# ylab-hi/ChimeraLM

Measured on AMD Instinct MI355X. Metric: reads/sec (whole node), 8192-bp reads batch=256, higher is better.
Workload: dtype fp16c

## Files before the change

chimeralm_amd/csrc/clm_api.hip:

```cpp
#include <cstdio>
#include <cstdlib>
#include <cmath>
#include <cstring>
#include <map>
#include <algorithm>
#include <string>
#include <vector>

#include "chimeralm_hip.h"
#include "clm_common.h"

using namespace clm;

namespace clm {
bool debug_flag(const char* name) {
    const char* e = std::getenv("CLM_DEBUG");
    if (!e) return false;
    const size_t n = std::strlen(name);
    for (const char* p = e; *p;) {
        const char* q = std::strchr(p, ',');
        const size_t len = q ? (size_t)(q - p) : std::strlen(p);
        if (len == n && std::strncmp(p, name, n) == 0) return true;
        p += len + (q ? 1 : 0);
    }
// ... 348 lines not shown
    *krev_out = nullptr;
    const int S = conv_segments_for(L);
    const int logn = S > 1 ? 14 : conv_logn_for(L);
    if (logn < 0 || L > h->cfg.max_seq_len)
        return fail(h, CLM_E_UNSUPPORTED, "sequence length " + std::to_string(L) + " tokens exceeds max_seq_len " +
                                              std::to_string(h->cfg.max_seq_len));
    const int key = S > 1 ? KEY_LONG : logn;
    FilterSet* fs = nullptr;
    for (auto& f : h->filters)
        if (f.key == key) fs = &f;
    const int N = 1 << logn;
    if (!fs) {
        HIPCHK(h, hipStreamSynchronize(st));
        FilterSet f;
        f.key = key;
        f.logn = logn;
        f.Lf = S > 1 ? h->cfg.max_seq_len : std::min(N / 2 + 1, h->cfg.max_seq_len);
        f.KS = S > 1 ? conv_segments_for(h->cfg.max_seq_len) : 1;
        DevBuf scratch;
        HIPCHK(h, scratch.alloc((size_t)D * N * sizeof(double2)));
        HIPCHK(h, f.tw.alloc((size_t)(N / 2) * sizeof(float2)));
        launch_twiddles(f.tw.get<float2>(), logn, st);
        for (int i = 0; i < NLAYER; ++i) {
            HIPCHK(h, f.ktime[i].alloc((size_t)f.Lf * D * 4));
            HIPCHK(h, f.kf[i].alloc((size_t)D * f.KS * N * sizeof(float2)));
            float* const kt = f.ktime[i].get<float>();
            float2* const kf = f.kf[i].get<float2>();
            const BlockF32& b = h->blk[i];
            launch_filter(b.pos_z, b.pos_t, b.f_w0, b.f_b0, b.f_freq, b.f_w2, b.f_b2, b.f_w4, b.f_b4, b.f_w6, b.deltas, kt, f.Lf, st);
            if (S == 1) {
                launch_filter_spectrum(kt, b.filt_bias, kf, scratch.get<double2>(), f.Lf, logn, 0, f.Lf, -1, st);
                if (logn == 14) {
                    HIPCHK(h, f.kfp[i].alloc((size_t)D * N * sizeof(float2)));
                    launch_spectrum_lanepack(kf, f.kfp[i].get<float2>(), 1, 0, st);
                }
            } else {
                DevBuf tmp;
                HIPCHK(h, tmp.alloc((size_t)D * N * sizeof(float2)));
                for (int j = 0; j < f.KS; ++j) {
                    launch_filter_spectrum(kt, b.filt_bias, tmp.get<float2>(), scratch.get<double2>(), f.Lf, logn, j * SEG_LEN,
                                           SEG_LEN, (j - 1) * SEG_LEN, st);
                    launch_spectrum_lanepack(tmp.get<float2>(), kf, f.KS, j, st);
                }
                HIPCHK(h, hipStreamSynchronize(st));
            }
        }
        HIPCHK(h, hipGetLastError());
        HIPCHK(h, hipStreamSynchronize(st));
        h->filters.push_back(std::move(f));
        fs = &h->filters.back();
    }
    if (conv_lone_tail(L)) {
        for (auto& r : fs->krev)
            if (r.L == L) *krev_out = &r;
        if (!*krev_out) {
            ReversedFilter r;
            r.L = L;
            r.stride = round_up(L, 8);
            for (int i = 0; i < NLAYER; ++i) {
                HIPCHK(h, r.p[i].alloc((size_t)D * r.stride * 4));
                launch_filter_reversed(fs->ktime[i].get<float>(), h->blk[i].filt_bias, r.p[i].get<float>(), L, r.stride, st);
            }
            fs->krev.push_back(std::move(r));
            *krev_out = &fs->krev.back();
        }
    }
    *out = fs;
// ... 442 lines not shown
extern "C" {

int clm_abi_version(void) { return CLM_ABI_VERSION; }

int clm_default_config(clm_config* c) {
    if (!c) return CLM_E_INVALID;
    std::memset(c, 0, sizeof(*c));
    c->struct_size = (int32_t)sizeof(clm_config);
    c->d_model = D; c->n_layer = NLAYER; c->d_inner = DI; c->vocab_rows = VOCAB; c->filter_order = FORDER;
    c->emb_dim = EMB; c->max_seq_len = 32770; c->head_hidden = HH; c->n_classes = NCLS;
    c->ln_eps = 1e-5f;
    c->precision = CLM_PREC_F32;
    c->chunk_reads = 256;
    return CLM_OK;
}

int clm_create(const clm_config* cfg, int device, clm_handle** out) {
    if (!cfg || !out) return fail<clm_handle>(nullptr, CLM_E_INVALID, "clm_create: null argument");
    if (cfg->struct_size != (int32_t)sizeof(clm_config)) return fail<clm_handle>(nullptr, CLM_E_INVALID, "clm_config size mismatch");
    if (cfg->d_model != D || cfg->n_layer != NLAYER || cfg->d_inner != DI || cfg->vocab_rows != VOCAB ||
        cfg->filter_order != FORDER || cfg->emb_dim != EMB || cfg->head_hidden != HH || cfg->n_classes != NCLS)
        return fail<clm_handle>(nullptr, CLM_E_UNSUPPORTED,
                                "only the HyenaDNA-small-32k + 512-wide attention-pooling head of chimeralm/models/lm.py is built");
    if (cfg->precision < CLM_PREC_F32 || cfg->precision > CLM_PREC_F16X3 || cfg->chunk_reads < 1 ||
        cfg->max_seq_len < 2)
        return fail<clm_handle>(nullptr, CLM_E_INVALID, "clm_create: bad precision / chunk_reads / max_seq_len");
    if (int rc = use_gfx950<clm_handle>(device, "clm_create")) return rc;
    clm_handle* h = new clm_handle();
    h->unfused_fp32 = debug_flag("unfused_fp32");
    h->no_idconv = debug_flag("no_idconv");
    h->no_lone_peel = debug_flag("no_lone_peel");
    if (debug_flag("conv_oneshot")) h->conv_flags |= CONV_ONESHOT;
    if (debug_flag("conv_no_xcd")) h->conv_flags |= CONV_NO_XCD;
    h->raw_z = debug_flag("raw_z");
    h->no_pad_skip = debug_flag("no_pad_skip");
    h->no_seg_skip = debug_flag("no_seg_skip");
    h->cfg = *cfg;
    if (cfg->precision == CLM_PREC_F16X3) {
        h->x3 = true;
        h->cfg.precision = CLM_PREC_F32;
        if (h->unfused_fp32) { delete h; return fail<clm_handle>(nullptr, CLM_E_UNSUPPORTED, "CLM_PREC_F16X3 exists in the fused tail kernels only (CLM_DEBUG=unfused_fp32 is set)"); }
    }
    h->device = device;
    if (hipHostMalloc((void**)&h->bad_ids, sizeof(int), hipHostMallocMapped) == hipSuccess) *h->bad_ids = 0;
    else h->bad_ids = nullptr;
    *out = h;
    return CLM_OK;
}

int clm_load_weight(clm_handle* h, const char* key, const void* data, int dtype, const int64_t* shape, int ndim) {
    if (!h || !key || !data || !shape || ndim < 1 || ndim > 4) return fail(h, CLM_E_INVALID, "clm_load_weight: bad argument");
    std::string ck;
    if (!canonical_key(key, ck)) return fail(h, CLM_E_INVALID, std::string("unknown weight key: ") + key);
    if (ck.find("implicit_filter.3.freq") != std::string::npos || ck.find("implicit_filter.5.freq") != std::string::npos)
        return CLM_OK;
    const KeySpec* spec = nullptr;
    static thread_local std::vector<KeySpec> specs;
    specs = expected_keys(h);
    for (auto& s : specs)
        if (s.key == ck) spec = &s;
    if (!spec) return fail(h, CLM_E_INVALID, std::string("unknown weight key: ") + key);
    std::vector<int64_t> shp(shape, shape + ndim);
    if (shp != spec->shape) {
        std::string got, want;
        for (auto v : shp) got += std::to_string(v) + ",";
        for (auto v : spec->shape) want += std::to_string(v) + ",";
// ... 434 lines not shown
```

chimeralm_amd/csrc/clm_common.h:

```cpp
#pragma once
#include <hip/hip_runtime.h>
#include <stdint.h>

#include <array>
#include <atomic>
#include <cstdio>
#include <map>
#include <string>
#include <type_traits>
#include <utility>
#include <vector>

#include "chimeralm_hip.h"

namespace clm {

constexpr int D = 256;
constexpr int D3 = 768;
constexpr int DI = 1024;
constexpr int XCDS = 8;
constexpr int NLAYER = 4;
constexpr int VOCAB = 16;
constexpr int FORDER = 64;
constexpr int EMB = 5;
// ... 387 lines not shown
    const float *n_g, *n_b, *n_w, *n_bias;
    const float4* n_fir;
    const float2* edge_read;
    void* n_z;
    const float *att_w1, *att_b1, *att_w2, *att_b2;
    float *scores, *partial;
    float* ws;
    int B, L, Lp, ntiles;
    float eps;
    const unsigned char* ylo;
    int zlo;
};
size_t lone_token_ws_floats(int B);
void launch_lone_token(int prec, const LoneTokenArgs& a, hipStream_t st);
void launch_tail16(int prec, const TailArgs& m, int next, hipStream_t st);
void tail16_dump_stamps();
void conv_dump_stamps();
size_t packed_weight_bytes(int prec, int n, int k);
void launch_pack_weight(int prec, const float* w, void* out, int n, int k, hipStream_t st);

constexpr int SEG_LEN = 8192;
int conv_logn_for(int L);
int conv_segments_for(int L);
bool conv_lone_tail(int L);
void launch_filter_reversed(const float* k , const float* dskip, float* krev, int L, int stride, hipStream_t st);
void launch_filter(const float* z , const float* t , const float* w0, const float* b0,
                   const float* freq, const float* w2, const float* b2, const float* w4, const float* b4,
                   const float* w6, const float* deltas, float* k_out , int L, hipStream_t st);
void launch_filter_spectrum(const float* k , const float* dskip , float2* kf,
                            double2* scratch, int L, int logn, int seg_off, int seg_len, int prev_off, hipStream_t st);
void launch_twiddles(float2* tw, int logn, hipStream_t st);
constexpr int CONV_ONESHOT = 1;
constexpr int CONV_NO_XCD = 2;
constexpr int CONV_GATED = 4;
void launch_hyena_conv(int prec, const void* z, void* y, const float2* kf, const float2* tw, const float* ktime,
                       const float* short_w, const float* short_b, int B, int L, int Lp, int logn,
                       const unsigned char* ids8, const float* ztab, hipStream_t st, int flags = 0,
                       const float2* kf_packed = nullptr ,
                       unsigned char* ylo = nullptr );
void launch_spectrum_lanepack(const float2* src, float2* dst, int KS, int j, hipStream_t st);
void launch_ztab(const float* emb, const float* g, const float* bta, const float* w, const float* bias, float* ztab,
                 float eps, hipStream_t st);

constexpr int SEG_DOT_THREADS = 512;
struct SegPrefix {
    const int* p0 = nullptr;
    const float2* tab = nullptr;
    int tab_segs = 0;
    const int* perm = nullptr;
    const float* dots_in = nullptr;
    float* dots_out = nullptr;
    int dots_segs = 0;
};
void launch_hyena_conv_seg(int prec, const void* z, void* y, const float2* kf, int KS ,
                           const float2* tw, const float* short_w,
                           const float* short_b, float2* gscratch, int B, int L, int Lp, int S,
                           const float* krev , int krev_stride,
                           const unsigned char* ids8 , const float* ztab,
                           hipStream_t st, int flags = 0, unsigned char* ylo = nullptr ,
                           const SegPrefix& pfx = SegPrefix{});
void launch_spectra_pair_form(float2* table, int S_T, hipStream_t st);

void launch_softmax_stats(const float* scores, float* stats , int B, int L, hipStream_t st);
constexpr int POOL_SPLIT = 16;
void launch_pool(const float* h, const float* g, const float* b, const float* scores, const float* stats,
                 float* partial , int B, int L, float eps, hipStream_t st);
struct HeadW {
    const float *w0t, *b0, *w3t, *b3, *w60t, *b60, *w63t, *b63, *wot, *bo;
};
void launch_head_mlp(const float* partial, const HeadW& hw, float* pooled_out, float* logits, int B, hipStream_t st);
constexpr int POOL_PSTRIDE = 264;
void launch_score_pool16(int prec, const float* h, const float* g, const float* bta, const void* w1, const float* b1,
                         const float* w2, const float* b2, float* scores, float* partial ,
// ... 34 lines not shown
```

chimeralm_amd/csrc/fft_core.h:

```cpp
#pragma once

#if defined(__HIPCC__)
#include <hip/hip_runtime.h>
#define CLM_HD __host__ __device__ __forceinline__
#define CLM_HDC __host__ __device__ constexpr
namespace clmfft {
using V2 = float __attribute__((ext_vector_type(2)));
CLM_HD V2 make_v2(float a, float b) { return V2{a, b}; }
CLM_HD V2 splat2(float a) { return V2{a, a}; }
}
#else
#include <cmath>
#define CLM_HD inline
#define CLM_HDC constexpr
struct float2 {
    float x, y;
};
static inline float2 make_float2(float x, float y) { return float2{x, y}; }
namespace clmfft {
struct V2 {
    float x, y;
};
inline V2 operator+(V2 a, V2 b) { return V2{a.x + b.x, a.y + b.y}; }
inline V2 operator-(V2 a, V2 b) { return V2{a.x - b.x, a.y - b.y}; }
// ... 155 lines not shown
        C t[16];
#pragma unroll
        for (int p = 0; p < 16; ++p) t[p] = v[p];
#pragma unroll
        for (int k1 = 0; k1 < 4; ++k1)
#pragma unroll
            for (int k2 = 0; k2 < 4; ++k2) v[4 * k1 + k2] = t[k1 + 4 * k2];
    }
};

template <bool INV>
struct Dft16HalfOut {
    template <class C>
    static CLM_HD void run(C* v) {
#pragma unroll
        for (int n1 = 0; n1 < 4; ++n1) dft4<INV>(v[n1], v[n1 + 4], v[n1 + 8], v[n1 + 12]);
#pragma unroll
        for (int n1 = 1; n1 < 4; ++n1)
#pragma unroll
            for (int k2 = 1; k2 < 4; ++k2) v[n1 + 4 * k2] = mul_w16<INV>(v[n1 + 4 * k2], n1 * k2);
        C x[9];
#pragma unroll
        for (int k2 = 0; k2 < 4; ++k2) {
            const C a0 = v[4 * k2], a1 = v[4 * k2 + 1], a2 = v[4 * k2 + 2], a3 = v[4 * k2 + 3];
            const C t0 = C::add(a0, a2), t1 = C::sub(a0, a2), t2 = C::add(a1, a3), t3 = C::template mul_mi<INV>(C::sub(a1, a3));
            x[k2] = C::add(t0, t2);
            x[4 + k2] = C::add(t1, t3);
            if (k2 == 0) x[8] = C::sub(t0, t2);
        }
#pragma unroll
        for (int q = 0; q < 9; ++q) v[q] = x[q];
    }
};

template <int R, class C>
CLM_HD void apply_twiddle_powers(C* v, C w1) {
    if (R >= 2) v[1] = C::mul(v[1], w1);
    if (R >= 4) {
        C w2 = C::mul(w1, w1), w3 = C::mul(w2, w1);
        v[2] = C::mul(v[2], w2);
        v[3] = C::mul(v[3], w3);
        if (R >= 8) {
            C w4 = C::mul(w2, w2), w5 = C::mul(w4, w1), w6 = C::mul(w4, w2), w7 = C::mul(w4, w3);
            v[4] = C::mul(v[4], w4);
            v[5] = C::mul(v[5], w5);
            v[6] = C::mul(v[6], w6);
            v[7] = C::mul(v[7], w7);
            if (R >= 16) {
                C w8 = C::mul(w4, w4);
                v[8] = C::mul(v[8], w8);
                v[9] = C::mul(v[9], C::mul(w8, w1));
                v[10] = C::mul(v[10], C::mul(w8, w2));
                v[11] = C::mul(v[11], C::mul(w8, w3));
                v[12] = C::mul(v[12], C::mul(w8, w4));
                v[13] = C::mul(v[13], C::mul(w8, w5));
                v[14] = C::mul(v[14], C::mul(w8, w6));
                v[15] = C::mul(v[15], C::mul(w8, w7));
            }
        }
    }
}

template <int LOGN>
struct Plan {
    static constexpr int N = 1 << LOGN;
    static constexpr int NPASS = (LOGN + 3) / 4;
// ... 31 lines not shown
```

chimeralm_amd/csrc/fft_passes.h:

```cpp
#pragma once
#include "fft_core.h"

namespace clmfft {

template <int LOGN, int R>
struct PassGeom {
    static constexpr int N = 1 << LOGN;
    static constexpr int NB = N / R;
    static constexpr int NT = Plan<LOGN>::NT;
    static constexpr int IT = (NB + NT - 1) / NT;
    static constexpr int NP = (IT + 1) / 2;
    static_assert(NP * R <= 16, "a thread holds at most 16 complex pairs");
    static CLM_HD int jba(int tid, int p) { return tid + (2 * p) * NT; }
    static CLM_HD int jbb(int tid, int p) { return tid + (2 * p + 1) * NT; }
    static constexpr bool FULL = (NB % NT == 0);
    static CLM_HD bool has_a(int tid, int p) { return FULL || jba(tid, p) < NB; }
    static CLM_HD bool has_b(int tid, int p) { return 2 * p + 1 < IT && (FULL || jbb(tid, p) < NB); }
    static_assert(NT % 32 == 0, "lane distance is a whole number of padding periods");
    static CLM_HDC int pb_of(int pa) { return pa + pad_offset(NT); }
};

template <int LOGN, int R>
CLM_HD void pass_load(const float* re, const float* im, Cx2* v, int tid) {
    using G = PassGeom<LOGN, R>;
// ... 103 lines not shown
        const bool ha = G::has_a(tid, p), hb = G::has_b(tid, p);
#pragma unroll
        for (int q = 0; q < R; ++q)
            kv[p * R + q] = pack2(ha ? kf[stockham_in<LOGN, R>(G::jba(tid, p), q)] : zero,
                                  hb ? kf[stockham_in<LOGN, R>(G::jbb(tid, p), q)] : zero);
    }
}

template <int LOGN, int R>
CLM_HD void spectrum_multiply_and_first_inverse_v(Cx2* v, int tid, const Cx2* kv, float tail_re = 0.f, float tail_im = 0.f) {
    using G = PassGeom<LOGN, R>;
    static_assert(((1 << LOGN) / R) % 2 == 0 && G::NT % 2 == 0, "bin parity == thread parity");
    const float sg = (tid & 1) ? -1.f : 1.f;
    const Cx2 tl{splat2(sg * tail_re), splat2(sg * tail_im)};
#pragma unroll
    for (int p = 0; p < G::NP; ++p) {
#pragma unroll
        for (int q = 0; q < R; ++q) v[p * R + q] = Cx2::mul(Cx2::add(v[p * R + q], tl), kv[p * R + q]);
        Dft<R, true>::run(v + p * R);
    }
}

template <int LOGN>
struct TwLayout {
    using P = Plan<LOGN>;
    static constexpr int NP16 = PassGeom<LOGN, 16>::NP;
    static constexpr int NPL = PassGeom<LOGN, P::LAST>::NP;
    static constexpr int fwd(int p) { return (p - 1) * NP16; }
    static constexpr int fwd_last() { return (P::NPASS - 2) * NP16; }
    static constexpr int inv(int p) { return (P::NPASS - 2) * NP16 + NPL + (p - 1) * NP16; }
    static constexpr int TOTAL = (2 * P::NPASS - 3) * NP16 + NPL;
};

}
```

chimeralm_amd/csrc/hyena_conv.hip:

```cpp
#include <cstdio>
#include <cstdlib>
#include <type_traits>
#include <vector>

#include "clm_common.h"
#include "fft_passes.h"

namespace clm {
using namespace clmfft;

__global__ __launch_bounds__(64) void filter_kernel(const float* __restrict__ z, const float* __restrict__ tn,
                                                    const float* __restrict__ w0, const float* __restrict__ b0,
                                                    const float* __restrict__ freq, const float* __restrict__ w2,
                                                    const float* __restrict__ b2, const float* __restrict__ w4,
                                                    const float* __restrict__ b4, const float* __restrict__ w6,
                                                    const float* __restrict__ deltas, float* __restrict__ k_out,
                                                    int L) {
    __shared__ double hbuf[2][FORDER];
    const int t = blockIdx.x, j = threadIdx.x;
    const double f = (double)freq[j];
    double acc = (double)b0[j];
#pragma unroll
    for (int e = 0; e < EMB; ++e) acc += (double)w0[j * EMB + e] * (double)z[(size_t)t * EMB + e];
    hbuf[0][j] = sin(f * acc);
// ... 615 lines not shown
            for (int e = 0; e < 8; ++e) {
                const bool ok = t0 + e < L;
                oA[e] = ok ? oA[e] * x0A[ch][e] : 0.f;
                oB[e] = ok ? oB[e] * x0B[ch][e] : 0.f;
            }
            ystore8<T, LO>(yA + t0, ylA + t0, oA);
            if (hasB) ystore8<T, LO>(yB + t0, ylB + t0, oB);
        }
    }
    if (tail && tid == TAIL_TID) {
        ystore1<T, LO>(yA + HALF, ylA + HALF, bre[pad_index(HALF)] * x0At);
        if (hasB) ystore1<T, LO>(yB + HALF, ylB + HALF, bim[pad_index(HALF)] * x0Bt);
    }
    CLM_STAMP_AT(11);
    if (STAMP && threadIdx.x == 0)
        stamps[((size_t)blockIdx.y * gridDim.x + blockIdx.x) * CONV_NSTAMP + 6] = __builtin_amdgcn_s_memrealtime();
#undef CLM_STAMP_AT
}


template <typename T, bool IDS, bool GATED = false, bool LO = false>
struct ConvGateRaw {
    Raw<T> r[GATED ? 1 : 2][2][GATED ? 1 : 2];
    T ztail[2][2];
    uint2 idd[2][2];
    unsigned short idp[2][2];
    unsigned char idt[2];
    uint4 g[2][2];
    T gtail[2];
    uint2 gl[2][2];
    unsigned char gltail[2];
};

template <typename T, bool IDS, bool GATED = false, bool LO = false>
__global__ __launch_bounds__(Plan<14>::NT) void hyena_conv_pers_kernel(
    const T* __restrict__ z, T* __restrict__ y, const float2* __restrict__ kf , const float2* __restrict__ tw,
    const float* __restrict__ ktime, const float* __restrict__ short_w, const float* __restrict__ short_b, int B, int L,
    int Lp, const unsigned char* __restrict__ ids8, const float* __restrict__ ztab, int use_xcd, unsigned char* __restrict__ ylo) {
    static_assert(!LO || std::is_same<T, f16_t>::value, "lo bytes exist in the compensated fp16 mode only");
    constexpr int LOGN = 14;
    using P = Plan<LOGN>;
    using TL = TwLayout<LOGN>;
    constexpr int N = P::N, NT = P::NT, LAST = P::LAST, HALF = N / 2, CH = 2;
    static_assert(HALF / 8 / NT == CH, "two 8-token chunks per thread");
    constexpr int TAIL_TID = HALF / 8 - 1 - (CH - 1) * NT;
    extern __shared__ __attribute__((aligned(16))) unsigned char smem[];
    float* bre = reinterpret_cast<float*>(smem);
    float* bim = bre + padded_size(N);
    float* gtail = bim + padded_size(N);
    float* zt = gtail + 4;

    const int tid = threadIdx.x;
    const int pairs = (B + 1) / 2, n_units = pairs * D;
    const bool tail = (L == HALF + 1);
    const bool xcd_order = use_xcd && (gridDim.x % XCDS) == 0;
    const int xcd = blockIdx.x % XCDS, wg_in_xcd = blockIdx.x / XCDS, wgs_per_xcd = gridDim.x / XCDS;
    const int first = xcd_order ? wg_in_xcd : (int)blockIdx.x, stride = xcd_order ? wgs_per_xcd : (int)gridDim.x;
    const int n_mine = xcd_order ? n_units / XCDS : n_units;
    auto unit_of = [&](int q, int& c, int& pair) {
        c = xcd_order ? XCDS * (q / pairs) + xcd : q / pairs;
        pair = q % pairs;
    };

    Cx2 wall[TL::TOTAL];
    {
        int ns = 16;
#pragma unroll
        for (int p = 1; p <= P::NPASS - 2; ++p) {
            pass_twiddles<LOGN, 16, false>(wall + TL::fwd(p), tid, ns, tw);
            ns *= 16;
        }
        pass_twiddles<LOGN, LAST, false>(wall + TL::fwd_last(), tid, ns, tw);
        ns = LAST;
#pragma unroll
        for (int p = 1; p <= P::NPASS - 1; ++p) {
            pass_twiddles<LOGN, 16, true>(wall + TL::inv(p), tid, ns, tw);
            ns *= 16;
        }
    }
    static_assert(!(GATED && IDS), "block 0 looks its rows up by token id: nothing to hand over");
    auto request_gate = [&](int q, ConvGateRaw<T, IDS, GATED, LO>& g, int ltid) {
        int c, pair;
        unit_of(q, c, pair);
        const int bA = 2 * pair, bB = (2 * pair + 1 < B) ? 2 * pair + 1 : bA;
        if constexpr (GATED) {
#pragma unroll
            for (int rd = 0; rd < 2; ++rd) {
                const T* row = z + ((size_t)(rd == 0 ? bA : bB) * D3 + D + c) * Lp;
                const unsigned char* rowl = zlo_row(z + (size_t)(rd == 0 ? bA : bB) * D3 * Lp, 1, c, Lp);
#pragma unroll
                for (int ch = 0; ch < CH; ++ch) {
                    const int t0 = 8 * (ltid + ch * NT);
                    g.g[ch][rd] = *reinterpret_cast<const uint4*>(row + (t0 < L ? t0 : 0));
                    if constexpr (LO) g.gl[ch][rd] = *reinterpret_cast<const uint2*>(rowl + (t0 < L ? t0 : 0));
                }
                g.gtail[rd] = row[(tail && ltid == TAIL_TID) ? HALF : 0];
                if constexpr (LO) g.gltail[rd] = rowl[(tail && ltid == TAIL_TID) ? HALF : 0];
            }
// ... 5 lines not shown
                for (int ch = 0; ch < CH; ++ch) {
                    const int t0 = 8 * (ltid + ch * NT);
                    const bool valid = t0 < L;
                    g.idd[ch][rd] = *reinterpret_cast<const uint2*>(ir + (valid ? t0 : 0));
                    g.idp[ch][rd] = *reinterpret_cast<const unsigned short*>(ir + ((valid && t0 > 0) ? t0 - 2 : 0));
                }
                g.idt[rd] = ir[(tail && ltid == TAIL_TID) ? HALF : 0];
            }
        } else {
#pragma unroll
            for (int rd = 0; rd < 2; ++rd) {
                const T* zr = z + (size_t)(rd == 0 ? bA : bB) * D3 * Lp;
#pragma unroll
                for (int a3 = 1; a3 < 3; ++a3) {
                    const T* row = zr + (size_t)(a3 * D + c) * Lp;
#pragma unroll
                    for (int ch = 0; ch < CH; ++ch) {
                        const int t0 = 8 * (ltid + ch * NT);
                        raw_load(g.r[ch][rd][a3 - 1], row, t0, t0 < L);
                    }
                    g.ztail[rd][a3 - 1] = row[(tail && ltid == TAIL_TID) ? HALF : 0];
                }
            }
        }
    };

    ConvGateRaw<T, IDS, GATED, LO> cur;
    request_gate(first < n_mine ? first : 0, cur, tid);

#pragma unroll 1
    for (int u = first; u < n_mine; u += stride) {
        int ltid = tid;
        asm volatile("" : "+v"(ltid));
#pragma unroll
        for (int i = 0; i < TL::TOTAL; ++i)
            asm volatile("" : "+v"(wall[i].re.x), "+v"(wall[i].re.y), "+v"(wall[i].im.x), "+v"(wall[i].im.y));
        int c, pair;
        unit_of(u, c, pair);
        const int bA = 2 * pair, bB = 2 * pair + 1;
        const bool hasB = bB < B;
        const float4* kfc = reinterpret_cast<const float4*>(kf) + (size_t)c * (N / 2);
        float sw[3][3], sb[3];
#pragma unroll
        for (int q = 0; q < 3; ++q) {
#pragma unroll
            for (int e = 0; e < 3; ++e) sw[q][e] = short_w[(q * D + c) * 3 + e];
            sb[q] = short_b[q * D + c];
        }
        if constexpr (IDS) {
            if (ltid < 48) zt[ltid] = ztab[(size_t)(ltid & 15) * D3 + (ltid >> 4) * D + c];
            __syncthreads();
        }
        const bool full_unit = L >= HALF && hasB;
        auto phase_a = [&](auto fullc) {
            constexpr bool FULL = decltype(fullc)::value;
            float gAt = 0.f, gBt = 0.f;
            if constexpr (GATED) {
#pragma unroll
                for (int ch = 0; ch < CH; ++ch) {
                    const int t0 = 8 * (ltid + ch * NT);
                    float gA[8], gB[8];
                    cvt8<T>(cur.g[ch][0], gA);
                    cvt8<T>(cur.g[ch][1], gB);
                    if constexpr (LO) {
                        add_lo8(cur.gl[ch][0], gA);
                        add_lo8(cur.gl[ch][1], gB);
                    }
                    if constexpr (!FULL) {
#pragma unroll
// ... 30 lines not shown
                fir3_pair(xa[1], xb[1], sw[1][0], sw[1][1], sw[1][2], sb[1], x1, x1b);
                fir3_pair(xa[2], xb[2], sw[2][0], sw[2][1], sw[2][2], sb[2], v, vb);
#pragma unroll
                for (int e = 0; e < 8; ++e) {
                    gA[e] = (FULL || t0 + e < L) ? v[e] * x1[e] : 0.f;
                    gB[e] = (FULL || (hasB && t0 + e < L)) ? vb[e] * x1b[e] : 0.f;
                }
                lds_store8(bre + pad_index(t0), gA);
                lds_store8(bim + pad_index(t0), gB);
                if (ch == CH - 1 && tail && ltid == TAIL_TID) {
                    float ta[3] = {0.f, 0.f, 0.f}, tb[3] = {0.f, 0.f, 0.f};
#pragma unroll
                    for (int a3 = 1; a3 < 3; ++a3) {
                        const float za = IDS ? zt[a3 * 16 + (cur.idt[0] & 15)] : to_float(cur.ztail[0][a3 - 1]);
                        const float zb = IDS ? zt[a3 * 16 + (cur.idt[1] & 15)] : to_float(cur.ztail[1][a3 - 1]);
                        ta[a3] = sb[a3] + sw[a3][0] * xa[a3][8] + sw[a3][1] * xa[a3][9] + sw[a3][2] * za;
                        tb[a3] = sb[a3] + sw[a3][0] * xb[a3][8] + sw[a3][1] * xb[a3][9] + sw[a3][2] * zb;
                    }
                    gAt = ta[1] * ta[2];
                    gBt = hasB ? tb[1] * tb[2] : 0.f;
                }
            }
            if (tail && ltid == TAIL_TID) {
                gtail[0] = gAt;
                gtail[1] = gBt;
            }
            }
        };
        if (full_unit) phase_a(std::true_type{});
        else phase_a(std::false_type{});
        __syncthreads();

        Cx2 v[16];
        {
            int Ns = 1;
#pragma unroll
            for (int p = 0; p < P::NPASS - 1; ++p) {
                if (p == 0) {
                    pass_first_lower<LOGN>(bre, bim, v, ltid);
                } else {
                    pass_load<LOGN, 16>(bre, bim, v, ltid);
                    pass_compute_w<LOGN, 16, false>(v, ltid, true, wall + TL::fwd(p));
                }
                __syncthreads();
                pass_store<LOGN, 16>(bre, bim, v, ltid, Ns);
                __syncthreads();
                Ns *= 16;
            }
        }
        {
            Cx2 kv[16];
#pragma unroll
            for (int e = 0; e < 16; ++e) {
                const float4 q4 = kfc[e * NT + ltid];
                kv[e] = Cx2{make_v2(q4.x, q4.y), make_v2(q4.z, q4.w)};
            }
            pass_load<LOGN, LAST>(bre, bim, v, ltid);
            pass_compute_w<LOGN, LAST, false>(v, ltid, true, wall + TL::fwd_last());
            spectrum_multiply_and_first_inverse_v<LOGN, LAST>(v, ltid, kv, tail ? gtail[0] : 0.f, tail ? gtail[1] : 0.f);
        }
        __syncthreads();
        pass_store<LOGN, LAST>(bre, bim, v, ltid, 1);
        __syncthreads();
        {
            int Ns = LAST;
#pragma unroll
            for (int p = 1; p < P::NPASS - 1; ++p) {
                pass_load<LOGN, 16>(bre, bim, v, ltid);
                pass_compute_w<LOGN, 16, true>(v, ltid, true, wall + TL::inv(p));
                __syncthreads();
                pass_store<LOGN, 16>(bre, bim, v, ltid, Ns);
                __syncthreads();
                Ns *= 16;
            }
        }
        Raw<T> x0r[CH][2];
        T x0tail[2];
        uint2 x0l[CH][2];
        unsigned char x0ltail[2] = {0, 0};
        const T* zA = z + (size_t)bA * D3 * Lp;
        const T* zB = z + (size_t)(hasB ? bB : bA) * D3 * Lp;
        if constexpr (GATED) {
#pragma unroll
            for (int rd = 0; rd < 2; ++rd) {
                const T* row = (rd == 0 ? zA : zB) + (size_t)c * Lp;
                const unsigned char* rowl = zlo_row(rd == 0 ? zA : zB, 0, c, Lp);
#pragma unroll
                for (int ch = 0; ch < CH; ++ch) {
                    const int t0 = 8 * (ltid + ch * NT);
                    x0r[ch][rd].d = *reinterpret_cast<const uint4*>(row + (t0 < L ? t0 : 0));
                    if constexpr (LO) x0l[ch][rd] = *reinterpret_cast<const uint2*>(rowl + (t0 < L ? t0 : 0));
                }
                x0tail[rd] = row[(tail && ltid == TAIL_TID) ? HALF : 0];
                if constexpr (LO) x0ltail[rd] = rowl[(tail && ltid == TAIL_TID) ? HALF : 0];
            }
        } else if constexpr (!IDS) {
#pragma unroll
            for (int rd = 0; rd < 2; ++rd) {
                const T* row = (rd == 0 ? zA : zB) + (size_t)c * Lp;
#pragma unroll
                for (int ch = 0; ch < CH; ++ch) {
                    const int t0 = 8 * (ltid + ch * NT);
                    raw_load(x0r[ch][rd], row, t0, t0 < L);
                }
                x0tail[rd] = row[(tail && ltid == TAIL_TID) ? HALF : 0];
            }
        }
        ConvGateRaw<T, IDS, GATED, LO> nxt;
        {
            const int un = u + stride;
            request_gate(un < n_mine ? un : u, nxt, ltid);
        }
        pass_load<LOGN, 16>(bre, bim, v, ltid);
        pass_compute_last_inverse_lower<LOGN>(v, ltid, wall + TL::inv(P::NPASS - 1));
        __syncthreads();
        pass_store_lower<LOGN>(bre, bim, v, ltid, tail);
        __syncthreads();

        auto phase_c = [&](auto fullc) {
            constexpr bool FULL = decltype(fullc)::value;
            T* yA = y + ((size_t)bA * D + c) * Lp;
            T* yB = y + ((size_t)(hasB ? bB : bA) * D + c) * Lp;
            unsigned char* ylA = LO ? ylo + ((size_t)bA * D + c) * Lp : nullptr;
            unsigned char* ylB = LO ? ylo + ((size_t)(hasB ? bB : bA) * D + c) * Lp : nullptr;
#pragma unroll
            for (int ch = 0; ch < CH; ++ch) {
                const int t0 = 8 * (ltid + ch * NT);
                const bool valid = FULL ? true : t0 < L, validB = FULL ? true : (valid && hasB);
                float xa[10] = {}, xb[10] = {}, x0a[8], x0b[8];
                if constexpr (GATED) {
                    cvt8<T>(x0r[ch][0].d, x0a);
                    cvt8<T>(x0r[ch][1].d, x0b);
                    if constexpr (LO) {
                        add_lo8(x0l[ch][0], x0a);
                        add_lo8(x0l[ch][1], x0b);
                    }
                } else if constexpr (IDS) {
                    float xa3[3][10], xb3[3][10];
#pragma unroll
                    for (int rd = 0; rd < 2; ++rd)
                        asm volatile("" : "+v"(cur.idd[ch][rd].x), "+v"(cur.idd[ch][rd].y), "+v"(cur.idp[ch][rd]));
                    ids_decode<true, 1>(cur.idd[ch][0], cur.idp[ch][0], t0, valid, zt, xa3);
                    ids_decode<true, 1>(cur.idd[ch][1], cur.idp[ch][1], t0, validB, zt, xb3);
#pragma unroll
                    for (int e = 0; e < 10; ++e) xa[e] = xa3[0][e], xb[e] = xb3[0][e];
                } else {
                    raw_decode(x0r[ch][0], t0, valid, xa);
// ... 9 lines not shown
                        oA[0] -= kl * gtail[0];
                        oB[0] -= kl * gtail[1];
                    }
#pragma unroll
                    for (int e = 0; e < 8; ++e) {
                        const bool ok = FULL || t0 + e < L;
                        oA[e] = ok ? oA[e] * x0a[e] : 0.f;
                        oB[e] = ok ? oB[e] * x0b[e] : 0.f;
                    }
                    ystore8<T, LO>(yA + t0, ylA + t0, oA);
                    if (hasB) ystore8<T, LO>(yB + t0, ylB + t0, oB);
                }
                if (ch == CH - 1 && tail && ltid == TAIL_TID) {
                    float za = IDS ? zt[cur.idt[0] & 15] : to_float(x0tail[0]);
                    float zb = IDS ? zt[cur.idt[1] & 15] : to_float(x0tail[1]);
                    if constexpr (GATED && LO) za += lo1b(x0ltail[0]), zb += lo1b(x0ltail[1]);
                    const float x0At = GATED ? za : sb[0] + sw[0][0] * xa[8] + sw[0][1] * xa[9] + sw[0][2] * za;
                    const float x0Bt = GATED ? zb : sb[0] + sw[0][0] * xb[8] + sw[0][1] * xb[9] + sw[0][2] * zb;
                    ystore1<T, LO>(yA + HALF, ylA + HALF, bre[pad_index(HALF)] * x0At);
                    if (hasB) ystore1<T, LO>(yB + HALF, ylB + HALF, bim[pad_index(HALF)] * x0Bt);
                }
            }
        };
        if (full_unit) phase_c(std::true_type{});
        else phase_c(std::false_type{});
        cur = nxt;
        __syncthreads();
    }
}

template <typename T, bool IDS, bool GATED = false, bool LO = false>
static void launch_conv_pers_inst(const void* z, void* y, const float2* kf, const float2* tw, const float* ktime,
                                  const float* short_w, const float* short_b, int B, int L, int Lp, const unsigned char* ids8,
                                  const float* ztab, int use_xcd, hipStream_t st, unsigned char* ylo = nullptr) {
    using P = Plan<14>;
    constexpr size_t lds = (size_t)2 * padded_size(P::N) * sizeof(float) + 256;
    static const int cus = [] {
        int dev = 0, n = 256;
        if (hipGetDevice(&dev) == hipSuccess) (void)hipDeviceGetAttribute(&n, hipDeviceAttributeMultiprocessorCount, dev);
        return n > 0 ? n : 256;
    }();
    const int n_units = ((B + 1) / 2) * D;
    dim3 grid(n_units < cus ? n_units : cus), block(P::NT);
    launch_lds<hyena_conv_pers_kernel<T, IDS, GATED, LO>>(grid, block, lds, st, reinterpret_cast<const T*>(z), reinterpret_cast<T*>(y), kf,
                                                         tw, ktime, short_w, short_b, B, L, Lp, ids8, ztab, use_xcd, ylo);
}


typedef unsigned v4u32 __attribute__((vector_size(16)));
__device__ __forceinline__ __amdgpu_buffer_rsrc_t make_rsrc(const void* p, size_t bytes) {
    const unsigned long long a = reinterpret_cast<unsigned long long>(p);
    const unsigned lo = __builtin_amdgcn_readfirstlane((unsigned)a), hi = __builtin_amdgcn_readfirstlane((unsigned)(a >> 32));
    void* q = reinterpret_cast<void*>(((unsigned long long)hi << 32) | lo);
    return __builtin_amdgcn_make_buffer_rsrc(q, 0, __builtin_amdgcn_readfirstlane((int)bytes), 0x00020000);
}

__global__ __launch_bounds__(512) void spectrum_lanepack_kernel(const float2* __restrict__ src, float4* __restrict__ dst, int KS, int j) {
    constexpr int N = 16384, NT = 512, LAST = Plan<14>::LAST;
    static_assert(LAST == 4 && Plan<14>::NT == NT, "pair geometry of the 16384-point plan");
    const int c = blockIdx.x, t = threadIdx.x;
    const float2* s = src + (size_t)c * N;
    float4* d = dst + ((size_t)c * KS + j) * (N / 2);
#pragma unroll
    for (int e = 0; e < 16; ++e) {
        const int ka = 2 * (e / LAST) + (N / LAST / NT) * (e % LAST);
        const float2 a = s[t + NT * ka], b = s[t + NT * (ka + 1)];
        d[e * NT + t] = make_float4(a.x, b.x, a.y, b.y);
    }
}
void launch_spectrum_lanepack(const float2* src, float2* dst, int KS, int j, hipStream_t st) {
    hipLaunchKernelGGL(spectrum_lanepack_kernel, dim3(D), dim3(512), 0, st, src, reinterpret_cast<float4*>(dst), KS, j);
}

template <typename T, bool LONE, bool IDS, bool GATED = false, bool LO = false>
__global__ __launch_bounds__(Plan<14>::NT) void hyena_conv_seg_kernel(
    const T* __restrict__ z, T* __restrict__ y, const float2* __restrict__ kf ,
    int KS, const float2* __restrict__ tw, const float* __restrict__ short_w, const float* __restrict__ short_b,
    float2* __restrict__ gscratch , int B, int L, int Lp, int S,
    const float* __restrict__ krev , int krev_stride,
    const unsigned char* __restrict__ ids8 , const float* __restrict__ ztab , int use_xcd,
    unsigned char* __restrict__ ylo, const SegPrefix pfx) {
    static_assert(!LO || std::is_same<T, f16_t>::value, "lo bytes exist in the compensated fp16 mode only");
    constexpr int LOGN = 14;
    using P = Plan<LOGN>;
    using TL = TwLayout<LOGN>;
    constexpr int N = P::N, NT = P::NT, LAST = P::LAST, HALF = N / 2, CH = HALF / 8 / NT;
    static_assert(HALF == SEG_LEN && CH == 2, "segment = half transform");
    static_assert(NT == SEG_DOT_THREADS, "one partial dot product per thread in SegPrefix::dots");
    extern __shared__ __attribute__((aligned(16))) unsigned char smem[];
    float* bre = reinterpret_cast<float*>(smem);
    float* bim = bre + padded_size(N);

    const int tid = threadIdx.x;
    const int pairs = (B + 1) / 2, xcd = blockIdx.x % XCDS, slot = blockIdx.x / XCDS;
    const int c = use_xcd ? XCDS * (slot / pairs) + xcd : (int)blockIdx.x / pairs, pair = use_xcd ? slot % pairs : (int)blockIdx.x % pairs;
    const bool hasB = 2 * pair + 1 < B;
    const int bA = pfx.perm ? pfx.perm[2 * pair] : 2 * pair;
    const int bB = hasB ? (pfx.perm ? pfx.perm[2 * pair + 1] : 2 * pair + 1) : bA;
    const T* zA = z + (size_t)bA * D3 * Lp;
    const T* zB = z + (size_t)(hasB ? bB : bA) * D3 * Lp;
    T* yA = y + ((size_t)bA * D + c) * Lp;
    T* yB = y + ((size_t)(hasB ? bB : bA) * D + c) * Lp;
    unsigned char* ylA = LO ? ylo + ((size_t)bA * D + c) * Lp : nullptr;
    unsigned char* ylB = LO ? ylo + ((size_t)(hasB ? bB : bA) * D + c) * Lp : nullptr;
// ... 588 lines not shown
            launch_lds<hyena_conv_kernel<LOGN, T, true>>(grid, block, lds, st, zt, yt, kf, tw, ktime, short_w, short_b, B, L, Lp,
                                                          s_conv_stamp_buf, no_ids, no_tab, (unsigned char*)nullptr);
            return;
        }
    }
    launch_lds<hyena_conv_kernel<LOGN, T, false, false, false, LO>>(grid, block, lds, st, zt, yt, kf, tw, ktime, short_w, short_b, B, L,
                                                                    Lp, no_stamps, no_ids, no_tab, ylo);
}

template <int LOGN>
static void launch_conv_p(int prec, const void* z, void* y, const float2* kf, const float2* tw, const float* ktime,
                          const float* short_w, const float* short_b, int B, int L, int Lp, const unsigned char* ids8,
                          const float* ztab, hipStream_t st, bool gated, unsigned char* ylo) {
    if (prec == PREC_F16C && ylo)
        launch_conv_t<LOGN, f16_t, true>(z, y, kf, tw, ktime, short_w, short_b, B, L, Lp, ids8, ztab, st, gated, ylo);
    else if (prec == PREC_F32)
        launch_conv_t<LOGN, float>(z, y, kf, tw, ktime, short_w, short_b, B, L, Lp, ids8, ztab, st, false);
    else if (prec == PREC_BF16)
        launch_conv_t<LOGN, bf16_t>(z, y, kf, tw, ktime, short_w, short_b, B, L, Lp, ids8, ztab, st, gated);
    else
        launch_conv_t<LOGN, f16_t>(z, y, kf, tw, ktime, short_w, short_b, B, L, Lp, ids8, ztab, st, gated);
}

void launch_hyena_conv(int prec, const void* z, void* y, const float2* kf, const float2* tw, const float* ktime,
                       const float* short_w, const float* short_b, int B, int L, int Lp, int logn,
                       const unsigned char* ids8, const float* ztab, hipStream_t st, int flags, const float2* kf_packed,
                       unsigned char* ylo) {
    static const bool stamp = debug_flag("stamp");
    const bool ids = ids8 != nullptr && ztab != nullptr;
    const bool gated = (flags & CONV_GATED) != 0 && !ids;
    const bool lo = prec == PREC_F16C && ylo != nullptr;
    if (logn == 14 && !(flags & CONV_ONESHOT) && !(stamp && !gated) && kf_packed) {
        kf = kf_packed;
        const int xcd = !(flags & CONV_NO_XCD);
        if (prec == PREC_F32) {
            if (ids) launch_conv_pers_inst<float, true>(nullptr, y, kf, tw, ktime, short_w, short_b, B, L, Lp, ids8, ztab, xcd, st);
            else launch_conv_pers_inst<float, false>(z, y, kf, tw, ktime, short_w, short_b, B, L, Lp, nullptr, nullptr, xcd, st);
        } else if (prec == PREC_BF16) {
            if (ids) launch_conv_pers_inst<bf16_t, true>(nullptr, y, kf, tw, ktime, short_w, short_b, B, L, Lp, ids8, ztab, xcd, st);
            else if (gated) launch_conv_pers_inst<bf16_t, false, true>(z, y, kf, tw, ktime, short_w, short_b, B, L, Lp, nullptr, nullptr, xcd, st);
            else launch_conv_pers_inst<bf16_t, false>(z, y, kf, tw, ktime, short_w, short_b, B, L, Lp, nullptr, nullptr, xcd, st);
        } else if (lo) {
            if (ids) launch_conv_pers_inst<f16_t, true, false, true>(nullptr, y, kf, tw, ktime, short_w, short_b, B, L, Lp, ids8, ztab, xcd, st, ylo);
            else if (gated) launch_conv_pers_inst<f16_t, false, true, true>(z, y, kf, tw, ktime, short_w, short_b, B, L, Lp, nullptr, nullptr, xcd, st, ylo);
            else launch_conv_pers_inst<f16_t, false, false, true>(z, y, kf, tw, ktime, short_w, short_b, B, L, Lp, nullptr, nullptr, xcd, st, ylo);
        } else {
            if (ids) launch_conv_pers_inst<f16_t, true>(nullptr, y, kf, tw, ktime, short_w, short_b, B, L, Lp, ids8, ztab, xcd, st);
            else if (gated) launch_conv_pers_inst<f16_t, false, true>(z, y, kf, tw, ktime, short_w, short_b, B, L, Lp, nullptr, nullptr, xcd, st);
            else launch_conv_pers_inst<f16_t, false>(z, y, kf, tw, ktime, short_w, short_b, B, L, Lp, nullptr, nullptr, xcd, st);
        }
        return;
    }
#define CLM_CONV_CASE(n) \
    case n: launch_conv_p<n>(prec, z, y, kf, tw, ktime, short_w, short_b, B, L, Lp, ids8, ztab, st, gated, ylo); break;
    switch (logn) {
        CLM_CONV_CASE(8)
        CLM_CONV_CASE(9)
        CLM_CONV_CASE(10)
        CLM_CONV_CASE(11)
        CLM_CONV_CASE(12)
        CLM_CONV_CASE(13)
        CLM_CONV_CASE(14)
        default: break;
    }
#undef CLM_CONV_CASE
}

// ... 2 lines not shown
```

Before: 8254.

## Restructure 16384-point persistent conv FFT into radix-32 passes

Replaces the four radix-16 passes plus lower pass in the persistent Hyena conv kernel with a 16×32×32 factorization. Two radix-32 passes run forward, the spectrum multiply is fused with the first inverse radix-32 butterfly, then one more radix-32 pass runs before the existing last inverse pass. The lane-packed filter spectrum is reordered to match the new layout. The aim is fewer LDS round trips and barriers, and far fewer twiddle registers than the old per-pass twiddle array. The cost is more registers per radix-32 butterfly and new inline-asm lane-crossing code. The old path stays available behind a debug flag.

```diff
diff --git a/chimeralm_amd/csrc/clm_api.hip b/chimeralm_amd/csrc/clm_api.hip
--- a/chimeralm_amd/csrc/clm_api.hip
+++ b/chimeralm_amd/csrc/clm_api.hip
@@ -404,7 +404,7 @@
                 launch_filter_spectrum(kt, b.filt_bias, kf, scratch.get<double2>(), f.Lf, logn, 0, f.Lf, -1, st);
                 if (logn == 14) {
                     HIPCHK(h, f.kfp[i].alloc((size_t)D * N * sizeof(float2)));
-                    launch_spectrum_lanepack(kf, f.kfp[i].get<float2>(), 1, 0, st);
+                    launch_spectrum_lanepack(kf, f.kfp[i].get<float2>(), 1, 0, st, !(h->conv_flags & CONV_4PASS));
                 }
             } else {
                 DevBuf tmp;
@@ -913,6 +913,7 @@
     h->no_lone_peel = debug_flag("no_lone_peel");
     if (debug_flag("conv_oneshot")) h->conv_flags |= CONV_ONESHOT;
     if (debug_flag("conv_no_xcd")) h->conv_flags |= CONV_NO_XCD;
+    if (debug_flag("conv_4pass")) h->conv_flags |= CONV_4PASS;
     h->raw_z = debug_flag("raw_z");
     h->no_pad_skip = debug_flag("no_pad_skip");
     h->no_seg_skip = debug_flag("no_seg_skip");
diff --git a/chimeralm_amd/csrc/clm_common.h b/chimeralm_amd/csrc/clm_common.h
--- a/chimeralm_amd/csrc/clm_common.h
+++ b/chimeralm_amd/csrc/clm_common.h
@@ -443,13 +443,14 @@
 void launch_twiddles(float2* tw, int logn, hipStream_t st);
 constexpr int CONV_ONESHOT = 1;
 constexpr int CONV_NO_XCD = 2;
+constexpr int CONV_4PASS = 8;
 constexpr int CONV_GATED = 4;
 void launch_hyena_conv(int prec, const void* z, void* y, const float2* kf, const float2* tw, const float* ktime,
                        const float* short_w, const float* short_b, int B, int L, int Lp, int logn,
                        const unsigned char* ids8, const float* ztab, hipStream_t st, int flags = 0,
                        const float2* kf_packed = nullptr ,
                        unsigned char* ylo = nullptr );
-void launch_spectrum_lanepack(const float2* src, float2* dst, int KS, int j, hipStream_t st);
+void launch_spectrum_lanepack(const float2* src, float2* dst, int KS, int j, hipStream_t st, bool plan3 = false);
 void launch_ztab(const float* emb, const float* g, const float* bta, const float* w, const float* bias, float* ztab,
                  float eps, hipStream_t st);
 
diff --git a/chimeralm_amd/csrc/fft_core.h b/chimeralm_amd/csrc/fft_core.h
--- a/chimeralm_amd/csrc/fft_core.h
+++ b/chimeralm_amd/csrc/fft_core.h
@@ -211,6 +211,117 @@
         for (int q = 0; q < 9; ++q) v[q] = x[q];
     }
 };
+
+
+CLM_HD V2 cross_lanes(V2 a) {
+#if defined(__HIP_DEVICE_COMPILE__)
+    V2 r;
+    asm("v_pk_add_f32 %0, %1, %1 op_sel:[0,1] op_sel_hi:[0,1] neg_hi:[0,1]" : "=v"(r) : "v"(a));
+    return r;
+#else
+    return make_v2(a.x + a.y, a.x - a.y);
+#endif
+}
+CLM_HD Cx2 cross_lanes(Cx2 a) { return Cx2{cross_lanes(a.re), cross_lanes(a.im)}; }
+
+CLM_HD Cx2 mul_lane_b(Cx2 a, float cr, float ci) {
+#if defined(__HIP_DEVICE_COMPILE__)
+    float t;
+    asm("v_mul_f32 %2, %4, %1\n\tv_mul_f32 %1, %3, %1\n\tv_fma_f32 %1, %0, %4, %1\n\tv_fma_f32 %0, %0, %3, -%2"
+        : "+v"(a.re.y), "+v"(a.im.y), "=&v"(t)
+        : "s"(cr), "s"(ci));
+#else
+    const float r = a.re.y * cr - a.im.y * ci, i = a.re.y * ci + a.im.y * cr;
+    a.re.y = r;
+    a.im.y = i;
+#endif
+    return a;
+}
+template <bool INV>
+CLM_HD void w32_const(int j, float& cx, float& sy) {
+    const float c1 = 0.98078528040323044913f, c2 = 0.92387953251128673848f, c3 = 0.83146961230254523708f,
+                c4 = 0.70710678118654752440f, c5 = 0.55557023301960222474f, c6 = 0.38268343236508978178f,
+                c7 = 0.19509032201612826785f;
+    switch (j) {
+        case 1: cx = c1; sy = c7; break;
+        case 2: cx = c2; sy = c6; break;
+        case 3: cx = c3; sy = c5; break;
+        case 4: cx = c4; sy = c4; break;
+        case 5: cx = c5; sy = c3; break;
+        case 6: cx = c6; sy = c2; break;
+        case 7: cx = c7; sy = c1; break;
+        case 9: cx = -c7; sy = c1; break;
+        case 10: cx = -c6; sy = c2; break;
+        case 11: cx = -c5; sy = c3; break;
+        case 12: cx = -c4; sy = c4; break;
+        case 13: cx = -c3; sy = c5; break;
+        case 14: cx = -c2; sy = c6; break;
+        default: cx = -c1; sy = c7; break;
+    }
+    sy = INV ? sy : -sy;
+}
+
+template <bool INV>
+struct Dft<32, INV> {
+    static CLM_HD void run(Cx2* v) {
+        v[0] = cross_lanes(v[0]);
+#pragma unroll
+        for (int j = 1; j < 16; ++j) {
+            if (j == 8) {
+                const Cx2 a = v[j];
+                v[j].re = make_v2(a.re.x + a.re.y, INV ? a.im.y - a.im.x : a.im.x - a.im.y);
+                v[j].im = make_v2(a.im.x + a.im.y, INV ? a.re.x - a.re.y : a.re.y - a.re.x);
+            } else {
+                float cx, sy;
+                w32_const<INV>(j, cx, sy);
+                v[j] = mul_lane_b(cross_lanes(v[j]), cx, sy);
+            }
+        }
+        Dft<16, INV>::run(v);
+    }
+};
+template <bool INV>
+struct Dft32Dit {
+    static CLM_HD void run(Cx2* v) {
+        Dft<16, INV>::run(v);
+        v[0] = cross_lanes(v[0]);
+#pragma unroll
+        for (int k = 1; k < 16; ++k) {
+            if (k == 8) {
+                const Cx2 a = v[k];
+                v[k].re = INV ? make_v2(a.re.x - a.im.y, a.re.x + a.im.y) : make_v2(a.re.x + a.im.y, a.re.x - a.im.y);
+                v[k].im = INV ? make_v2(a.im.x + a.re.y, a.im.x - a.re.y) : make_v2(a.im.x - a.re.y, a.im.x + a.re.y);
+            } else {
+                float cx, sy;
+                w32_const<INV>(k, cx, sy);
+                v[k] = cross_lanes(mul_lane_b(v[k], cx, sy));
+            }
+        }
+    }
+};
+
+CLM_HD void apply_twiddle_powers32(Cx2* v, Cx2 t0, Cx2 t1) {
+    const Cx2 p1{splat2(t1.re.x), splat2(t1.im.x)};
+    const Cx2 p2 = Cx2::mul(p1, p1), p4 = Cx2::mul(p2, p2), p8 = Cx2::mul(p4, p4);
+    const Cx2 t2 = Cx2::mul(t0, p2), t3 = Cx2::mul(t1, p2);
+    const Cx2 t4 = Cx2::mul(t0, p4), t5 = Cx2::mul(t1, p4), t6 = Cx2::mul(t2, p4), t7 = Cx2::mul(t3, p4);
+    v[0] = Cx2::mul(v[0], t0);
+    v[1] = Cx2::mul(v[1], t1);
+    v[2] = Cx2::mul(v[2], t2);
+    v[3] = Cx2::mul(v[3], t3);
+    v[4] = Cx2::mul(v[4], t4);
+    v[5] = Cx2::mul(v[5], t5);
+    v[6] = Cx2::mul(v[6], t6);
+    v[7] = Cx2::mul(v[7], t7);
+    v[8] = Cx2::mul(v[8], Cx2::mul(t0, p8));
+    v[9] = Cx2::mul(v[9], Cx2::mul(t1, p8));
+    v[10] = Cx2::mul(v[10], Cx2::mul(t2, p8));
+    v[11] = Cx2::mul(v[11], Cx2::mul(t3, p8));
+    v[12] = Cx2::mul(v[12], Cx2::mul(t4, p8));
+    v[13] = Cx2::mul(v[13], Cx2::mul(t5, p8));
+    v[14] = Cx2::mul(v[14], Cx2::mul(t6, p8));
+    v[15] = Cx2::mul(v[15], Cx2::mul(t7, p8));
+}
 
 template <int R, class C>
 CLM_HD void apply_twiddle_powers(C* v, C w1) {
diff --git a/chimeralm_amd/csrc/fft_passes.h b/chimeralm_amd/csrc/fft_passes.h
--- a/chimeralm_amd/csrc/fft_passes.h
+++ b/chimeralm_amd/csrc/fft_passes.h
@@ -159,4 +159,89 @@
     static constexpr int TOTAL = (2 * P::NPASS - 3) * NP16 + NPL;
 };
 
-}
+template <int LOGN>
+struct Plan3 {
+    static constexpr int N = 1 << LOGN;
+    static constexpr int NT = Plan<LOGN>::NT;
+    static constexpr int NB = N / 32;
+    static_assert(LOGN == 14 && NB == NT, "16 * 32 * 32 with one radix-32 butterfly per thread");
+    static constexpr int NS_F1 = 16, NS_F2 = 512, NS_I1 = 32, NS_I2 = 1024;
+};
+
+struct Tw32 {
+    Cx2 t0, t1;
+};
+struct TwSet3 {
+    Tw32 f1, f2, i1;
+    Cx2 i2;
+};
+
+template <int LOGN, bool INV>
+CLM_HD Tw32 pass32_twiddles(int tid, int Ns, const float2* tw) {
+    constexpr int N = 1 << LOGN;
+    const int m = (tid & (Ns - 1)) * (N / (Ns * 32));
+    auto at = [&](int i) { return INV ? cconj(tw[i]) : tw[i]; };
+    return Tw32{pack2(make_float2(1.f, 0.f), at(m)), pack2(at(2 * m), at(3 * m))};
+}
+
+template <int LOGN>
+CLM_HD void pass32_load(const float* re, const float* im, Cx2* v, int tid) {
+    using P = Plan3<LOGN>;
+    const float* ra = re + pad_index(tid);
+    const float* ia = im + pad_index(tid);
+    constexpr int dB = pad_offset(P::NB);
+#pragma unroll
+    for (int j = 0; j < 16; ++j) {
+        const int off = pad_offset(2 * j * P::NB);
+        v[j].re = make_v2(ra[off], ra[off + dB]);
+        v[j].im = make_v2(ia[off], ia[off + dB]);
+    }
+}
+
+template <bool INV>
+CLM_HD void pass32_compute(Cx2* v, const Tw32& w) {
+    apply_twiddle_powers32(v, w.t0, w.t1);
+    Dft32Dit<INV>::run(v);
+}
+
+template <int LOGN, int Ns>
+CLM_HD void pass32_store(float* re, float* im, const Cx2* v, int tid) {
+    static_assert(Ns == 16 || Ns % 32 == 0, "base (mod 32) + offset (mod 32) stays inside one padding period");
+    const int k = tid & (Ns - 1);
+    const int pa = pad_index((tid - k) * 32 + k);
+#pragma unroll
+    for (int q = 0; q < 16; ++q) {
+        const int oa = pad_offset(q * Ns), ob = pad_offset((q + 16) * Ns);
+        re[pa + oa] = v[q].re.x, re[pa + ob] = v[q].re.y;
+        im[pa + oa] = v[q].im.x, im[pa + ob] = v[q].im.y;
+    }
+}
+
+template <int LOGN>
+CLM_HD void pass32_store_first(float* re, float* im, const Cx2* v, int tid) {
+    const int pa = pad_index(tid * 32);
+#pragma unroll
+    for (int k = 0; k < 16; ++k) {
+        re[pa + 2 * k] = v[k].re.x, re[pa + 2 * k + 1] = v[k].re.y;
+        im[pa + 2 * k] = v[k].im.x, im[pa + 2 * k + 1] = v[k].im.y;
+    }
+}
+
+template <int LOGN>
+CLM_HD void spectrum_fetch32(Cx2* kv, int tid, const float2* kf) {
+    using P = Plan3<LOGN>;
+#pragma unroll
+    for (int k = 0; k < 16; ++k) kv[k] = pack2(kf[tid + P::NB * k], kf[tid + P::NB * (k + 16)]);
+}
+
+template <int LOGN>
+CLM_HD void spectrum_multiply_and_first_inverse32(Cx2* v, int tid, const Cx2* kv, float tail_re = 0.f, float tail_im = 0.f) {
+    static_assert(Plan3<LOGN>::NB % 2 == 0, "bin parity == thread parity");
+    const float sg = (tid & 1) ? -1.f : 1.f;
+    const Cx2 tl{splat2(sg * tail_re), splat2(sg * tail_im)};
+#pragma unroll
+    for (int q = 0; q < 16; ++q) v[q] = Cx2::mul(Cx2::add(v[q], tl), kv[q]);
+    Dft<32, true>::run(v);
+}
+
+}
diff --git a/chimeralm_amd/csrc/hyena_conv.hip b/chimeralm_amd/csrc/hyena_conv.hip
--- a/chimeralm_amd/csrc/hyena_conv.hip
+++ b/chimeralm_amd/csrc/hyena_conv.hip
@@ -671,7 +671,7 @@
     unsigned char gltail[2];
 };
 
-template <typename T, bool IDS, bool GATED = false, bool LO = false>
+template <typename T, bool IDS, bool GATED = false, bool LO = false, bool P4 = false>
 __global__ __launch_bounds__(Plan<14>::NT) void hyena_conv_pers_kernel(
     const T* __restrict__ z, T* __restrict__ y, const float2* __restrict__ kf , const float2* __restrict__ tw,
     const float* __restrict__ ktime, const float* __restrict__ short_w, const float* __restrict__ short_b, int B, int L,
@@ -701,8 +701,15 @@
         pair = q % pairs;
     };
 
-    Cx2 wall[TL::TOTAL];
-    {
+    Cx2 wall[P4 ? TL::TOTAL : 1];
+    TwSet3 w3;
+    if constexpr (!P4) {
+        using P3 = Plan3<LOGN>;
+        w3.f1 = pass32_twiddles<LOGN, false>(tid, P3::NS_F1, tw);
+        w3.f2 = pass32_twiddles<LOGN, false>(tid, P3::NS_F2, tw);
+        w3.i1 = pass32_twiddles<LOGN, true>(tid, P3::NS_I1, tw);
+        pass_twiddles<LOGN, 16, true>(&w3.i2, tid, P3::NS_I2, tw);
+    } else {
         int ns = 16;
 #pragma unroll
         for (int p = 1; p <= P::NPASS - 2; ++p) {
@@ -774,9 +781,13 @@
     for (int u = first; u < n_mine; u += stride) {
         int ltid = tid;
         asm volatile("" : "+v"(ltid));
-#pragma unroll
-        for (int i = 0; i < TL::TOTAL; ++i)
-            asm volatile("" : "+v"(wall[i].re.x), "+v"(wall[i].re.y), "+v"(wall[i].im.x), "+v"(wall[i].im.y));
+        auto opaque = [](Cx2& w) { asm volatile("" : "+v"(w.re.x), "+v"(w.re.y), "+v"(w.im.x), "+v"(w.im.y)); };
+        if constexpr (P4) {
+#pragma unroll
+            for (int i = 0; i < TL::TOTAL; ++i) opaque(wall[i]);
+        } else {
+            opaque(w3.f1.t0), opaque(w3.f1.t1), opaque(w3.f2.t0), opaque(w3.f2.t1), opaque(w3.i1.t0), opaque(w3.i1.t1), opaque(w3.i2);
+        }
         int c, pair;
         unit_of(u, c, pair);
         const int bA = 2 * pair, bB = 2 * pair + 1;
@@ -873,6 +884,37 @@
         __syncthreads();
 
         Cx2 v[16];
+        if constexpr (!P4) {
+            using P3 = Plan3<LOGN>;
+            pass_first_lower<LOGN>(bre, bim, v, ltid);
+            __syncthreads();
+            pass_store<LOGN, 16>(bre, bim, v, ltid, 1);
+            __syncthreads();
+            pass32_load<LOGN>(bre, bim, v, ltid);
+            pass32_compute<false>(v, w3.f1);
+            __syncthreads();
+            pass32_store<LOGN, P3::NS_F1>(bre, bim, v, ltid);
+            __syncthreads();
+            {
+                Cx2 kv[16];
+#pragma unroll
+                for (int e = 0; e < 16; ++e) {
+                    const float4 q4 = kfc[e * NT + ltid];
+                    kv[e] = Cx2{make_v2(q4.x, q4.y), make_v2(q4.z, q4.w)};
+                }
+                pass32_load<LOGN>(bre, bim, v, ltid);
+                pass32_compute<false>(v, w3.f2);
+                spectrum_multiply_and_first_inverse32<LOGN>(v, ltid, kv, tail ? gtail[0] : 0.f, tail ? gtail[1] : 0.f);
+            }
+            __syncthreads();
+            pass32_store_first<LOGN>(bre, bim, v, ltid);
+            __syncthreads();
+            pass32_load<LOGN>(bre, bim, v, ltid);
+            pass32_compute<true>(v, w3.i1);
+            __syncthreads();
+            pass32_store<LOGN, P3::NS_I1>(bre, bim, v, ltid);
+            __syncthreads();
+        } else {
         {
             int Ns = 1;
 #pragma unroll
@@ -915,6 +957,7 @@
                 Ns *= 16;
             }
         }
+        }
         Raw<T> x0r[CH][2];
         T x0tail[2];
         uint2 x0l[CH][2];
@@ -953,7 +996,8 @@
             request_gate(un < n_mine ? un : u, nxt, ltid);
         }
         pass_load<LOGN, 16>(bre, bim, v, ltid);
-        pass_compute_last_inverse_lower<LOGN>(v, ltid, wall + TL::inv(P::NPASS - 1));
+        if constexpr (P4) pass_compute_last_inverse_lower<LOGN>(v, ltid, wall + TL::inv(P::NPASS - 1));
+        else pass_compute_last_inverse_lower<LOGN>(v, ltid, &w3.i2);
         __syncthreads();
         pass_store_lower<LOGN>(bre, bim, v, ltid, tail);
         __syncthreads();
@@ -1029,7 +1073,8 @@
 template <typename T, bool IDS, bool GATED = false, bool LO = false>
 static void launch_conv_pers_inst(const void* z, void* y, const float2* kf, const float2* tw, const float* ktime,
                                   const float* short_w, const float* short_b, int B, int L, int Lp, const unsigned char* ids8,
-                                  const float* ztab, int use_xcd, hipStream_t st, unsigned char* ylo = nullptr) {
+                                  const float* ztab, int use_xcd , hipStream_t st,
+                                  unsigned char* ylo = nullptr) {
     using P = Plan<14>;
     constexpr size_t lds = (size_t)2 * padded_size(P::N) * sizeof(float) + 256;
     static const int cus = [] {
@@ -1039,8 +1084,12 @@
     }();
     const int n_units = ((B + 1) / 2) * D;
     dim3 grid(n_units < cus ? n_units : cus), block(P::NT);
-    launch_lds<hyena_conv_pers_kernel<T, IDS, GATED, LO>>(grid, block, lds, st, reinterpret_cast<const T*>(z), reinterpret_cast<T*>(y), kf,
-                                                         tw, ktime, short_w, short_b, B, L, Lp, ids8, ztab, use_xcd, ylo);
+    if (use_xcd & 2)
+        launch_lds<hyena_conv_pers_kernel<T, IDS, GATED, LO, true>>(grid, block, lds, st, reinterpret_cast<const T*>(z), reinterpret_cast<T*>(y),
+                                                                   kf, tw, ktime, short_w, short_b, B, L, Lp, ids8, ztab, use_xcd & 1, ylo);
+    else
+        launch_lds<hyena_conv_pers_kernel<T, IDS, GATED, LO>>(grid, block, lds, st, reinterpret_cast<const T*>(z), reinterpret_cast<T*>(y), kf,
+                                                             tw, ktime, short_w, short_b, B, L, Lp, ids8, ztab, use_xcd, ylo);
 }
 
 
@@ -1052,7 +1101,8 @@
     return __builtin_amdgcn_make_buffer_rsrc(q, 0, __builtin_amdgcn_readfirstlane((int)bytes), 0x00020000);
 }
 
-__global__ __launch_bounds__(512) void spectrum_lanepack_kernel(const float2* __restrict__ src, float4* __restrict__ dst, int KS, int j) {
+__global__ __launch_bounds__(512) void spectrum_lanepack_kernel(const float2* __restrict__ src, float4* __restrict__ dst, int KS, int j,
+                                                                int plan3) {
     constexpr int N = 16384, NT = 512, LAST = Plan<14>::LAST;
     static_assert(LAST == 4 && Plan<14>::NT == NT, "pair geometry of the 16384-point plan");
     const int c = blockIdx.x, t = threadIdx.x;
@@ -1060,13 +1110,13 @@
     float4* d = dst + ((size_t)c * KS + j) * (N / 2);
 #pragma unroll
     for (int e = 0; e < 16; ++e) {
-        const int ka = 2 * (e / LAST) + (N / LAST / NT) * (e % LAST);
-        const float2 a = s[t + NT * ka], b = s[t + NT * (ka + 1)];
+        const int ka = plan3 ? e : 2 * (e / LAST) + (N / LAST / NT) * (e % LAST), kb = plan3 ? e + 16 : ka + 1;
+        const float2 a = s[t + NT * ka], b = s[t + NT * kb];
         d[e * NT + t] = make_float4(a.x, b.x, a.y, b.y);
     }
 }
-void launch_spectrum_lanepack(const float2* src, float2* dst, int KS, int j, hipStream_t st) {
-    hipLaunchKernelGGL(spectrum_lanepack_kernel, dim3(D), dim3(512), 0, st, src, reinterpret_cast<float4*>(dst), KS, j);
+void launch_spectrum_lanepack(const float2* src, float2* dst, int KS, int j, hipStream_t st, bool plan3) {
+    hipLaunchKernelGGL(spectrum_lanepack_kernel, dim3(D), dim3(512), 0, st, src, reinterpret_cast<float4*>(dst), KS, j, plan3 ? 1 : 0);
 }
 
 template <typename T, bool LONE, bool IDS, bool GATED = false, bool LO = false>
@@ -1721,7 +1771,7 @@
     const bool lo = prec == PREC_F16C && ylo != nullptr;
     if (logn == 14 && !(flags & CONV_ONESHOT) && !(stamp && !gated) && kf_packed) {
         kf = kf_packed;
-        const int xcd = !(flags & CONV_NO_XCD);
+        const int xcd = (!(flags & CONV_NO_XCD) ? 1 : 0) | ((flags & CONV_4PASS) ? 2 : 0);
         if (prec == PREC_F32) {
             if (ids) launch_conv_pers_inst<float, true>(nullptr, y, kf, tw, ktime, short_w, short_b, B, L, Lp, ids8, ztab, xcd, st);
             else launch_conv_pers_inst<float, false>(z, y, kf, tw, ktime, short_w, short_b, B, L, Lp, nullptr, nullptr, xcd, st);
```

Result: no change. 8443 (median of 6 runs) (+2.3%).
